# cmusphinx/pocketsphinx

Hardware: NVIDIA H100
Metric: frames/sec senone-eval+Viterbi (higher is better)
Workload: dtype f32->i16/i32

## Files before the change

### include/psb200.h

```cpp
#ifndef PSB200_H
#define PSB200_H

#include <stddef.h>
#include <stdint.h>

#ifdef __cplusplus
extern "C" {
#endif

#define PSB_ABI_VERSION 2

typedef enum psb_status_e {
    PSB_OK = 0,
    PSB_ERR_ARG = -1,
    PSB_ERR_CUDA = -2,
    PSB_ERR_NOMEM = -3,
    PSB_ERR_STATE = -4
} psb_status_t;

enum { PSB_KIND_PTM = 0, PSB_KIND_SEMI = 1, PSB_KIND_MS = 2 };

#define PSB_MAX_FEAT 8
#define PSB_MAX_TOPN 8
#define PSB_HMM_MAX_NSTATE 5
// ... 6 lines not shown
typedef struct psb_model_desc_s {
    int32_t kind, n_sen, n_mgau, n_feat, n_density, topn;
    int32_t featlen[PSB_MAX_FEAT];
    int32_t ds_ratio;
    int32_t aw;
    int32_t logadd_ms_size, logadd_ms_zero;
    int32_t on_device;
    const float *mean, *var, *det;
    const uint8_t *mixw, *mixw_cb;
    const int32_t *sen2cb;
    const uint8_t *logadd8;
    const uint32_t *logadd_ms;
    const uint8_t *topn_beam;
    int32_t fixed_point;
} psb_model_desc_t;

typedef struct psb_model_s psb_model_t;

int psb_model_create(const psb_model_desc_t *desc, int device, psb_model_t **out);
void psb_model_free(psb_model_t *m);
int psb_model_update_gaussians(psb_model_t *m, const float *mean, const float *var, const float *det);
int psb_model_n_sen(const psb_model_t *m);
int psb_model_device(const psb_model_t *m);

typedef struct psb_scorer_s psb_scorer_t;

int psb_scorer_create(psb_model_t *m, int32_t n_hist, psb_scorer_t **out);
void psb_scorer_free(psb_scorer_t *s);
int psb_scorer_reset(psb_scorer_t *s);
int psb_scorer_set_frame_idx(psb_scorer_t *s, int32_t frame_idx);
int32_t psb_scorer_get_frame_idx(const psb_scorer_t *s);
int psb_scorer_frame_eval(psb_scorer_t *s, int16_t *senscr, const uint8_t *senone_active,
                          int32_t n_senone_active, const float *const *feat, int32_t frame,
                          int32_t compallsen);

typedef struct psb_batch_s psb_batch_t;

int psb_batch_create(psb_model_t *m, int32_t max_utts, int64_t max_frames, psb_batch_t **out);
void psb_batch_free(psb_batch_t *b);
int psb_batch_score_host(psb_batch_t *b, const float *feats, const int32_t *utt_off,
                         int32_t n_utt, int16_t *senscr);
int psb_batch_score_device(psb_batch_t *b, const float *d_feats, const int32_t *utt_off,
                           int32_t n_utt, int16_t *d_senscr);
int psb_batch_sync(psb_batch_t *b);
int16_t *psb_batch_senscr_device(psb_batch_t *b);
int psb_batch_last_kernel_ms(psb_batch_t *b, float *out3);
int psb_batch_event_record(psb_batch_t *b, int slot);
int psb_batch_event_elapsed_ms(psb_batch_t *b, float *ms);
int psb_batch_tc_check(psb_batch_t *b, float *ratio, int32_t *max_candidates, int64_t *stats4);
#define PSB_TC_N_COUNTERS 15
int psb_batch_tc_counters(psb_batch_t *b, int64_t *out, int32_t n);
#define PSB_MS_PLAN_N 14
int psb_batch_ms_plan(psb_batch_t *b, int64_t total_frames, int64_t *out, int32_t n);
#define PSB_TM_PLAN_N 5
int psb_batch_tm_plan(psb_batch_t *b, int64_t total_frames, int64_t *out, int32_t n);
int psb_batch_get_topn(psb_batch_t *b, int32_t *rec, int64_t n_frames);

typedef struct psb_hmm_s {
    void *ctx;
    int32_t score[PSB_HMM_MAX_NSTATE];
    int32_t history[PSB_HMM_MAX_NSTATE];
    int32_t out_score;
    int32_t out_history;
    uint16_t ssid;
    uint16_t senid[PSB_HMM_MAX_NSTATE];
    int32_t bestscore;
    int16_t tmatid;
    int32_t frame;
    uint8_t mpx;
    uint8_t n_emit_state;
} psb_hmm_t;

typedef struct psb_hmmctx_s psb_hmmctx_t;

int psb_hmmctx_create(int32_t n_emit_state, const uint8_t *tp, int32_t n_tmat,
                      const uint16_t *sseq, int32_t n_sseq, int32_t n_sen, int device,
                      psb_hmmctx_t **out);
void psb_hmmctx_free(psb_hmmctx_t *c);

int psb_hmm_vit_eval_batch(psb_hmmctx_t *c, psb_hmm_t *hmms, int32_t n, const int16_t *senscr,
                           int32_t *best);
int psb_hmm_vit_eval_ptrs(psb_hmmctx_t *c, psb_hmm_t *const *hmms, int32_t n,
                          const int16_t *senscr, int32_t *best);

typedef struct psb_hmmset_s psb_hmmset_t;
int psb_hmmset_create(psb_hmmctx_t *c, int64_t n_max, int32_t n_seg_max, psb_hmmset_t **out);
void psb_hmmset_free(psb_hmmset_t *s);
int psb_hmmset_upload(psb_hmmset_t *s, const psb_hmm_t *hmms, int64_t n, const int64_t *seg_off,
                      int32_t n_seg);
int psb_hmmset_download(psb_hmmset_t *s, psb_hmm_t *hmms);
int psb_hmmset_eval_frames_device(psb_hmmset_t *s, const int16_t *d_senscr, const int64_t *d_row0,
                                  const int32_t *d_n_rows, int32_t n_frames, int32_t *d_best,
                                  float *ms);
int psb_hmmset_sweep_device(psb_hmmset_t *s, const int16_t *d_senscr, int64_t rows_total,
                            const int64_t *d_row0, const int32_t *d_n_rows, int32_t n_frames,
                            int32_t *d_best, float *ms);
int psb_hmmset_sweep_beam_device(psb_hmmset_t *s, const int16_t *d_senscr, int64_t rows_total,
                                 const int64_t *d_row0, const int32_t *d_n_rows, int32_t n_frames,
                                 int32_t frame0, int32_t beam, int32_t maxhmmpf, int32_t *d_best,
                                 int32_t *d_n_active, float *ms);
int psb_hmmset_use_batch_stream(psb_hmmset_t *s, psb_batch_t *b);
int psb_hmmset_snapshot(psb_hmmset_t *s);
int psb_hmmset_restore(psb_hmmset_t *s);
int psb_hmmset_eval_host(psb_hmmset_t *s, const int16_t *senscr, int32_t *best);

typedef struct psb_phoneloop_s psb_phoneloop_t;

// ... 256 lines not shown
```

### pocketsphinx_b200/api.py

```python
import ctypes as C

import numpy as np

from . import _lib
from ._lib import ModelDesc, PsbError, check, lib
from .model import PackedModel

KIND_ID = {"ptm": 0, "s2_semi": 1, "ms": 2}

HMM_DTYPE = np.dtype({
    "names": ["ctx", "score", "history", "out_score", "out_history", "ssid", "senid",
              "bestscore", "tmatid", "frame", "mpx", "n_emit_state"],
    "formats": ["<u8", ("<i4", 5), ("<i4", 5), "<i4", "<i4", "<u2", ("<u2", 5),
                "<i4", "<i2", "<i4", "u1", "u1"],
    "offsets": [0, 8, 28, 48, 52, 56, 58, 68, 72, 76, 80, 81],
    "itemsize": 88,
})


def _p(a):
    if a is None:
        return None
    if hasattr(a, "data_ptr"):
        return a.data_ptr()
# ... 131 lines not shown

    def set_pipeline(self, n):
        check(lib().psb_batch_set_pipeline(self.h, int(n)), "psb_batch_set_pipeline")

    def event_record(self, slot):
        check(lib().psb_batch_event_record(self.h, slot), "psb_batch_event_record")

    def event_elapsed_ms(self):
        ms = C.c_float()
        check(lib().psb_batch_event_elapsed_ms(self.h, C.byref(ms)), "psb_batch_event_elapsed_ms")
        return ms.value

    def run_phoneloop_device(self, phoneloop, utt_off, d_best_ptr=None, d_pen_ptr=None):
        utt_off = np.ascontiguousarray(utt_off, np.int32)
        check(lib().psb_phoneloop_run_device(phoneloop.h, self.senscr_device_ptr(), _p(utt_off), len(utt_off) - 1,
                                             d_best_ptr, d_pen_ptr, None, self.h), "psb_phoneloop_run_device")

    def decode_device(self, phoneloop, d_feats_ptr, utt_off):
        utt_off = np.ascontiguousarray(utt_off, np.int32)
        pb, pp = C.c_void_p(), C.c_void_p()
        check(lib().psb_decode_batch_device(self.h, phoneloop.h, d_feats_ptr, _p(utt_off), len(utt_off) - 1,
                                            C.byref(pb), C.byref(pp)), "psb_decode_batch_device")
        return pb.value, pp.value

    def get_topn(self, n_frames):
        rec = np.zeros((n_frames, self.model.pm.n_mgau * self.model.pm.n_feat, 4), np.int32)
        check(lib().psb_batch_get_topn(self.h, _p(rec), n_frames), "psb_batch_get_topn")
        return rec

    TC_COUNTERS = ("rows", "from_filter_alone", "exact_distances", "tie_fixups", "over_cap", "lane_over",
                   "fallback_listed", "fallback_all", "split_lists", "fail_gap", "fail_straddle", "fail_sign",
                   "fail_saturation", "tiles_per_cta", "ctas_per_pair")

    def tc_check(self):
        r, n = C.c_float(), C.c_int32()
        check(lib().psb_batch_tc_check(self.h, C.byref(r), C.byref(n), None), "psb_batch_tc_check")
        st = np.zeros(len(self.TC_COUNTERS), np.int64)
        check(lib().psb_batch_tc_counters(self.h, _p(st), len(st)), "psb_batch_tc_counters")
        self.tc_stats = {k: int(v) for k, v in zip(self.TC_COUNTERS, st)}
        return r.value, n.value

    MS_PLAN = ("tile", "fuse", "prefetch", "nt", "n_used", "all", "frames_per_cta", "tiles_x", "chunk", "n_chunks",
               "dist_bytes", "n_sm", "transposed", "tile_smem")

    def ms_plan(self, total_frames):
        v = np.zeros(len(self.MS_PLAN), np.int64)
        check(lib().psb_batch_ms_plan(self.h, int(total_frames), _p(v), len(v)), "psb_batch_ms_plan")
        return {k: int(x) for k, x in zip(self.MS_PLAN, v)}

    TM_TOPN = ("tc_filter", "ptm_scan", "ptm_scalar", "semi_split", "fixed")
    TM_SENONE = ("ptm_senone4", "ptm_senone_8b", "ptm_senone_4b", "semi_senone4", "semi_senone_8b", "semi_senone_4b")

    def tm_plan(self, total_frames):
        v = np.zeros(5, np.int64)
        check(lib().psb_batch_tm_plan(self.h, int(total_frames), _p(v), len(v)), "psb_batch_tm_plan")
        return dict(topn="+".join(n for i, n in enumerate(self.TM_TOPN) if int(v[0]) >> i & 1),
                    senone=self.TM_SENONE[int(v[1])], threads=int(v[2]), n_bsen=int(v[3]), smem=int(v[4]))

    def decode_host(self, phoneloop, feats, utt_off, want_senscr=False, best=None, pen=None, senscr=None):
        pm = self.model.pm
        utt_off = np.ascontiguousarray(utt_off, np.int32)
        total = int(utt_off[-1])
        if best is None:
            best = np.zeros(total, np.int32)
        if pen is None:
            pen = np.zeros((total, phoneloop.n_phones), np.int32)
        if want_senscr and senscr is None:
            senscr = np.zeros((total, pm.n_sen), np.int16)
        check(lib().psb_decode_batch_host(self.h, phoneloop.h, _p(feats), _p(utt_off), len(utt_off) - 1,
                                          _p(best), _p(pen), _p(senscr) if want_senscr else None),
              "psb_decode_batch_host")
        return (best, pen, senscr) if want_senscr else (best, pen)

    def decode_pcm_host(self, fe, phoneloop, pcm, samp_off, want_senscr=False):
        pm = self.model.pm
        pcm = np.ascontiguousarray(pcm, np.int16)
        samp_off = np.ascontiguousarray(samp_off, np.int64)
        n_utt = len(samp_off) - 1
        total = sum(fe.n_frames(int(samp_off[u + 1] - samp_off[u])) for u in range(n_utt))
        frame_off = np.zeros(n_utt + 1, np.int32)
        best = np.zeros(total, np.int32)
        pen = np.zeros((total, phoneloop.n_phones), np.int32)
        senscr = np.zeros((total, pm.n_sen), np.int16) if want_senscr else None
        check(lib().psb_decode_batch_pcm_host(self.h, fe.h, phoneloop.h, _p(pcm) if pcm.size else None, _p(samp_off), n_utt,
                                              _p(frame_off), _p(best), _p(pen), _p(senscr) if want_senscr else None),
              "psb_decode_batch_pcm_host")
        return (frame_off, best, pen, senscr) if want_senscr else (frame_off, best, pen)

    def score_pcm(self, fe, pcm, samp_off):
        pcm = np.ascontiguousarray(pcm, np.int16)
        samp_off = np.ascontiguousarray(samp_off, np.int64)
        n_utt = len(samp_off) - 1
        frame_off = np.zeros(n_utt + 1, np.int32)
        check(lib().psb_fe_process_host(fe.h, _p(pcm) if pcm.size else None, _p(samp_off), n_utt, None, None,
                                        _p(frame_off)), "psb_fe_process_host")
        if frame_off[-1]:
            self.score_device(lib().psb_fe_device_feats(fe.h), frame_off)
            self.sync()
        return frame_off

    def close(self):
        if self.h:
            lib().psb_batch_free(self.h)
            self.h = None


class HmmContext:

    def __init__(self, tp, sseq, n_sen, device=0):
        self.tp = np.ascontiguousarray(tp, np.uint8)
# ... 761 lines not shown
```

### pocketsphinx_b200/csrc/psb_ptm.cu

```cuda
#include "psb_gau.cuh"
#include "psb_internal.cuh"
#include "psb_tm.cuh"

#include <string.h>

#include <algorithm>
#include <numeric>

namespace {

constexpr int TOPN_WARPS = 4;
constexpr int MAX_NDW = 8;

template <int FL, bool SEMI>
__device__ __forceinline__ int gau_dist_fx(const float4 *__restrict__ r, const float (&x)[FL], int *dmin)
{
    constexpr int RECF = (1 + 2 * FL + 3) / 4 * 4;
    int rr[RECF];
#pragma unroll
    for (int q = 0; q < RECF / 4; ++q) {
        float4 v = r[q];
        rr[4 * q + 0] = __float_as_int(v.x); rr[4 * q + 1] = __float_as_int(v.y);
        rr[4 * q + 2] = __float_as_int(v.z); rr[4 * q + 3] = __float_as_int(v.w);
    }
// ... 544 lines not shown
    uint8_t *cb16 = tab + PSB_LOGADD8_N;
    int16_t *asc = reinterpret_cast<int16_t *>(cb16 + 16);
    const long long frame = blockIdx.x;
    const int tid = threadIdx.x;

    for (int i = tid; i < PSB_LOGADD8_N; i += blockDim.x) tab[i] = logadd_tab[i];
    if (FOURBIT && tid < 16) cb16[tid] = mixw_cb[tid];
    if (tid < n_feat) norm[tid] = PSB_WORST_SCORE;
    __syncthreads();
    ptm_norm_rows<false>(topn, frame, K, n_feat, nd, mixw_stride, norm, rowoff, nsc, nullptr);
    __syncthreads();

    int best = 0x7fffffff;
    for (int s = tid; s < n_sen; s += blockDim.x) {
        const int i0 = (int)sen2cb[s] * n_feat;
        const uint8_t *__restrict__ mw = mixw + (FOURBIT ? (s >> 1) : s);
        int ascore = 0;
        for (int f = 0; f < n_feat; ++f)
            ascore += ptm_mix<FOURBIT>(mw, rowoff[i0 + f], nsc[i0 + f], tab, cb16);
        best = min(best, ascore);
        asc[s] = (int16_t)ascore;
    }
    store_relative_to_best(best, red, asc, senscr + frame * n_sen, n_sen);
}

template <bool FOURBIT>
__global__ void __launch_bounds__(256)
semi_senone_kernel(const int4 *__restrict__ topn, const uint8_t *__restrict__ mixw,
                   const uint8_t *__restrict__ mixw_cb, const uint8_t *__restrict__ logadd_tab,
                   int16_t *__restrict__ senscr, int n_sen, int n_feat, int nd, int mixw_stride)
{
    extern __shared__ int smem_i[];
    uint4 *rowoff = reinterpret_cast<uint4 *>(smem_i);
    uint4 *nsc = rowoff + n_feat;
    uint8_t *tab = reinterpret_cast<uint8_t *>(nsc + n_feat);
    uint8_t *cb16 = tab + PSB_LOGADD8_N;
    __shared__ int cnt[PSB_MAX_FEAT];
    const long long frame = blockIdx.x;
    const int tid = threadIdx.x;
    for (int i = tid; i < PSB_LOGADD8_N; i += blockDim.x) tab[i] = logadd_tab[i];
    if (FOURBIT && tid < 16) cb16[tid] = mixw_cb[tid];
    semi_rows<false>(topn, frame, n_feat, nd, mixw_stride, rowoff, nsc, nullptr, cnt);
    __syncthreads();
    const int s = blockIdx.y * blockDim.x + tid;
    if (s >= n_sen) return;
    int16_t acc = 0;
    if (!FOURBIT || s < (n_sen & ~1)) {
        for (int f = 0; f < n_feat; ++f)
            acc = (int16_t)(acc + semi_mix<FOURBIT>(mixw, s, rowoff[f], nsc[f], cnt[f], tab, cb16));
    }
    senscr[frame * n_sen + s] = acc;
}

__global__ void __launch_bounds__(512)
ptm_senone4_kernel(const int4 *__restrict__ topn, const uint8_t *__restrict__ mixw,
                   const uint16_t *__restrict__ sen2cb, const int16_t *__restrict__ quadcb,
                   const int32_t *__restrict__ bsen, int n_bsen, const uint8_t *__restrict__ logadd_tab,
                   int16_t *__restrict__ senscr, int n_sen, int n_feat, int nd, int K, int mixw_stride)
{
    extern __shared__ int smem_i[];
    uint4 *rowoff = reinterpret_cast<uint4 *>(smem_i);
    uint4 *nsc = rowoff + K;
    uint4 *nvp = nsc + K;
    int *norm = reinterpret_cast<int *>(nvp + K);
    int *red = norm + 8;
    uint8_t *tab = reinterpret_cast<uint8_t *>(red + 32);
    int16_t *asc = reinterpret_cast<int16_t *>(tab + PSB_LOGADD8_N + 16);
    const long long frame = blockIdx.x;
    const int tid = threadIdx.x;

    for (int i = tid; i < PSB_LOGADD8_N; i += blockDim.x) tab[i] = logadd_tab[i];
    if (tid < n_feat) norm[tid] = PSB_WORST_SCORE;
    __syncthreads();
    ptm_norm_rows<true>(topn, frame, K, n_feat, nd, mixw_stride, norm, rowoff, nsc, nvp);
    __syncthreads();

    int best = 0x7fffffff;
    const int n_quads = (n_sen + 3) >> 2;
    for (int q = tid; q < n_quads; q += blockDim.x) {
        const int c = quadcb[q];
        if (c < 0) continue;
        const int s0 = q << 2, i0 = c * n_feat;
        const uint8_t *mw = mixw + s0;
        unsigned acc01 = 0u, acc23 = 0u;
        for (int f = 0; f < n_feat; ++f) {
            const uint4 ro = rowoff[i0 + f], nv = nvp[i0 + f];
            const unsigned w0 = *reinterpret_cast<const unsigned *>(mw + ro.x);
            const unsigned w1 = *reinterpret_cast<const unsigned *>(mw + ro.y);
            const unsigned w2 = *reinterpret_cast<const unsigned *>(mw + ro.z);
            const unsigned w3 = *reinterpret_cast<const unsigned *>(mw + ro.w);
            unsigned x01 = __byte_perm(w0, 0u, 0x4140) + nv.x;
            unsigned x23 = __byte_perm(w0, 0u, 0x4342) + nv.x;
            x01 = logadd8_16x2(tab, x01, w1, 0x4140, nv.y); x23 = logadd8_16x2(tab, x23, w1, 0x4342, nv.y);
            x01 = logadd8_16x2(tab, x01, w2, 0x4140, nv.z); x23 = logadd8_16x2(tab, x23, w2, 0x4342, nv.z);
            x01 = logadd8_16x2(tab, x01, w3, 0x4140, nv.w); x23 = logadd8_16x2(tab, x23, w3, 0x4342, nv.w);
            acc01 += x01;
            acc23 += x23;
        }
        const int unbias = n_feat * SEN_BIAS;
        const int a0 = (int)(acc01 & 0xffffu) - unbias, a1 = (int)(acc01 >> 16) - unbias;
        const int a2 = (int)(acc23 & 0xffffu) - unbias, a3 = (int)(acc23 >> 16) - unbias;
        best = min(min(best, a0), min(min(a1, a2), a3));
        *reinterpret_cast<short4 *>(asc + s0) = make_short4((short)a0, (short)a1, (short)a2, (short)a3);
    }
    for (int i = tid; i < n_bsen; i += blockDim.x) {
        const int s = bsen[i];
        const int i0 = (int)sen2cb[s] * n_feat;
        int ascore = 0;
        for (int f = 0; f < n_feat; ++f)
            ascore += ptm_mix<false>(mixw + s, rowoff[i0 + f], nsc[i0 + f], tab, nullptr);
        best = min(best, ascore);
        asc[s] = (int16_t)ascore;
    }
    store_relative_to_best(best, red, asc, senscr + frame * n_sen, n_sen);
}

template <int FL>
int launch_topnq(psb_batch_t *b, const int32_t *d_klist, int n_k, const GroupTabs &tabs, int n_groups,
                 const int32_t *d_featoff)
{
    psb_model_t *m = b->m;
    constexpr int RECF2 = (2 + 4 * FL + 3) / 4 * 4;
    const size_t smem = (size_t)(m->n_density / 2) * RECF2 * sizeof(float) + (size_t)QCAP * TOPN_WARPS * 32 * sizeof(float);
    auto kern = ptm_topnq_kernel<FL>;
    PSB_CUDA(cudaFuncSetAttribute(kern, cudaFuncAttributeMaxDynamicSharedMemorySize, (int)smem));
    dim3 grid(n_k, (n_groups + TOPN_WARPS - 1) / TOPN_WARPS);
    kern<<<grid, TOPN_WARPS * 32, smem, b->stream>>>(m->d_rec2, m->d_rec2_off, d_klist, b->d_featT, tabs, b->d_topn, n_groups,
                                                    m->n_density, m->n_feat, m->sumlen, d_featoff, m->K, m->ds_ratio);
    PSB_LAUNCH_CHECK();
    return PSB_OK;
}

template <int FL, bool SEMI>
int launch_topn(psb_batch_t *b, const int32_t *d_klist, int n_k, const GroupTabs &tabs, int n_groups,
                const int32_t *d_featoff)
{
    psb_model_t *m = b->m;
    if constexpr (!SEMI && FL <= 16) {
        if (!m->fixed_point) return launch_topnq<FL>(b, d_klist, n_k, tabs, n_groups, d_featoff);
    }
    auto kern = ptm_topn_kernel<FL, SEMI, true>;
    if constexpr (!SEMI && FL > 16) {
        if (!m->fixed_point) kern = ptm_topn_kernel<FL, false, false>;
    }
    size_t smem = (size_t)m->n_density * rec_floats(FL) * sizeof(float);
    PSB_CUDA(cudaFuncSetAttribute(kern, cudaFuncAttributeMaxDynamicSharedMemorySize, (int)smem));
    const int warps = (long long)n_k * ((n_groups + TOPN_WARPS - 1) / TOPN_WARPS) >= 4 * psb_sm_count(m->device) ? TOPN_WARPS : 1;
    dim3 grid(n_k, (n_groups + warps - 1) / warps);
    kern<<<grid, warps * 32, smem, b->stream>>>(m->d_rec, m->d_rec_off, d_klist, b->d_featT, tabs, b->d_topn, n_groups,
                                               m->n_density, m->n_feat, m->sumlen, d_featoff, m->K, m->ds_ratio,
                                               m->d_topn_beam);
    PSB_LAUNCH_CHECK();
    return PSB_OK;
}

__global__ void __launch_bounds__(512)
semi_senone4_kernel(const int4 *__restrict__ topn, const uint8_t *__restrict__ mixw,
                    const uint8_t *__restrict__ logadd_tab, int16_t *__restrict__ senscr, int n_sen, int n_feat, int nd,
                    int mixw_stride)
{
    __shared__ uint4 rowoff[PSB_MAX_FEAT], nvp[PSB_MAX_FEAT], nsc[PSB_MAX_FEAT];
    __shared__ int cnt[PSB_MAX_FEAT];
    __shared__ uint8_t tab[PSB_LOGADD8_N];
    const long long frame = blockIdx.x;
    const int tid = threadIdx.x;
    for (int i = tid; i < PSB_LOGADD8_N; i += blockDim.x) tab[i] = logadd_tab[i];
    semi_rows<true>(topn, frame, n_feat, nd, mixw_stride, rowoff, nsc, nvp, cnt);
    __syncthreads();
    int16_t *dst = senscr + frame * n_sen;
    const int n_quads = n_sen >> 2;
    for (int q = tid; q < n_quads; q += blockDim.x) {
        const int s0 = q << 2;
        const uint8_t *mw = mixw + s0;
        short a0 = 0, a1 = 0, a2 = 0, a3 = 0;
        for (int f = 0; f < n_feat; ++f) {
            const uint4 ro = rowoff[f], nv = nvp[f];
            const int n = cnt[f];
            const unsigned w0 = *reinterpret_cast<const unsigned *>(mw + ro.x);
            unsigned x01 = __byte_perm(w0, 0u, 0x4140) + nv.x, x23 = __byte_perm(w0, 0u, 0x4342) + nv.x;
            if (n > 1) {
                const unsigned w1 = *reinterpret_cast<const unsigned *>(mw + ro.y);
                x01 = logadd8_16x2(tab, x01, w1, 0x4140, nv.y); x23 = logadd8_16x2(tab, x23, w1, 0x4342, nv.y);
            }
            if (n > 2) {
                const unsigned w2 = *reinterpret_cast<const unsigned *>(mw + ro.z);
                x01 = logadd8_16x2(tab, x01, w2, 0x4140, nv.z); x23 = logadd8_16x2(tab, x23, w2, 0x4342, nv.z);
            }
            if (n > 3) {
                const unsigned w3 = *reinterpret_cast<const unsigned *>(mw + ro.w);
                x01 = logadd8_16x2(tab, x01, w3, 0x4140, nv.w); x23 = logadd8_16x2(tab, x23, w3, 0x4342, nv.w);
            }
            a0 = (short)(a0 + (int)(x01 & 0xffffu) - SEN_BIAS);
            a1 = (short)(a1 + (int)(x01 >> 16) - SEN_BIAS);
            a2 = (short)(a2 + (int)(x23 & 0xffffu) - SEN_BIAS);
            a3 = (short)(a3 + (int)(x23 >> 16) - SEN_BIAS);
        }
        if ((((uintptr_t)(dst + s0)) & 7) == 0)
            *reinterpret_cast<short4 *>(dst + s0) = make_short4(a0, a1, a2, a3);
        else { dst[s0] = a0; dst[s0 + 1] = a1; dst[s0 + 2] = a2; dst[s0 + 3] = a3; }
    }
    for (int s = (n_quads << 2) + tid; s < n_sen; s += blockDim.x) {
        int16_t acc = 0;
        for (int f = 0; f < n_feat; ++f)
            acc = (int16_t)(acc + semi_mix<false>(mixw, s, rowoff[f], nsc[f], cnt[f], tab, nullptr));
        dst[s] = acc;
    }
}

enum TmTopn { TOPN_TC_FILTER, TOPN_PTM_SCAN, TOPN_PTM_SCALAR, TOPN_SEMI_SPLIT, TOPN_FIXED };
enum TmSenone { SEN_PTM4, SEN_PTM_8B, SEN_PTM_4B, SEN_SEMI4, SEN_SEMI_8B, SEN_SEMI_4B };

bool topn_fl_instantiated(int fl)
{
    for (int v : {13, 12, 24, 3, 39, 1, 2, 4, 8, 16, 26, 32})
        if (fl == v) return true;
    return false;
}

constexpr size_t TM_SMEM_MAX = 227 * 1024;

struct TmPlan {
    unsigned topn_paths;
    bool semi_split;
    int senone;
    int threads;
    size_t smem;
};

int tm_plan(const psb_model_t *m, TmPlan *p)
{
    PSB_REQUIRE(m->kind == PSB_KIND_PTM || m->kind == PSB_KIND_SEMI, "psb_launch_ptm_batch: model is neither PTM nor semi-continuous");
    const bool semi = m->kind == PSB_KIND_SEMI;
    PSB_REQUIRE(m->topn == TOPN, "tied-mixture batch kernels are built for -topn 4 (got %d)", m->topn);
    PSB_REQUIRE(m->n_density % 32 == 0 && m->n_density <= 32 * MAX_NDW,
                "PTM batch kernels need n_density in {32..256, multiple of 32} (got %d)", m->n_density);
    const int K = m->K;
    const bool use_tc = !semi && psb_tc_usable(m);
    p->semi_split = semi && !m->fixed_point;
    p->topn_paths = 0;
    for (int f = 0; f < m->n_feat; ++f) {
        const int fl = m->featlen[f];
        if (use_tc) { p->topn_paths |= 1u << TOPN_TC_FILTER; continue; }
        if (!topn_fl_instantiated(fl)) {
            psb_set_error("no %s instantiation for stream length %d", p->semi_split ? "semi_dist_kernel" : "ptm_topn_kernel", fl);
            return PSB_ERR_ARG;
        }
        int path;
        if (p->semi_split) path = TOPN_SEMI_SPLIT;
        else if (m->fixed_point) path = TOPN_FIXED;
        else path = fl <= 16 ? TOPN_PTM_SCAN : TOPN_PTM_SCALAR;
        p->topn_paths |= 1u << path;
    }
    const bool bias_ok = (TOPN - 1) * m->logadd8_max < SEN_BIAS;
    if (semi) {
        PSB_REQUIRE(K <= 512, "semi_senone_kernel handles at most 512 streams (got %d)", K);
        if (!m->mixw_4bit && bias_ok) {
            p->senone = SEN_SEMI4; p->threads = 512; p->smem = 0;
        }
        else {
            p->senone = m->mixw_4bit ? SEN_SEMI_4B : SEN_SEMI_8B;
            p->threads = 256;
            p->smem = (size_t)K * 32 + PSB_LOGADD8_N + 16;
        }
        return PSB_OK;
    }
    PSB_REQUIRE(K <= 512, "ptm_senone_kernel handles at most 512 (codebook, stream) pairs (got %d)", K);
    PSB_REQUIRE((size_t)m->n_feat * m->n_density * m->mixw_stride < (1ull << 32), "mixture-weight table too large for 32-bit offsets");
    const size_t smem = (size_t)K * 32 + 8 * 4 + 32 * 4 + PSB_LOGADD8_N + 16 + (size_t)m->n_sen * 2;
    if (m->mixw_4bit || !bias_ok) {
        p->senone = m->mixw_4bit ? SEN_PTM_4B : SEN_PTM_8B;
        p->threads = 512;
        p->smem = smem;
    }
    else {
        const int n_quads = (m->n_sen + 3) / 4;
        const int iters = (n_quads + 511) / 512;
        p->senone = SEN_PTM4;
        p->threads = std::min(512, std::max(std::max(256, roundup(K, 32)), roundup((n_quads + iters - 1) / iters, 32)));
        p->smem = smem + 8 + (size_t)K * 16;
    }
    PSB_REQUIRE(p->smem <= TM_SMEM_MAX, "%d senones do not fit the PTM senone kernel's shared memory (%zu bytes, at most %zu)",
                m->n_sen, p->smem, TM_SMEM_MAX);
    return PSB_OK;
}

}

extern "C" int psb_batch_tm_plan(psb_batch_t *b, int64_t total_frames, int64_t *out, int32_t n)
{
    PSB_REQUIRE(b && (out || n == 0) && n >= 0 && total_frames >= 0, "psb_batch_tm_plan: bad argument");
    TmPlan p;
    const int rc = tm_plan(b->m, &p);
    if (rc) return rc;
    const int64_t v[PSB_TM_PLAN_N] = {p.topn_paths, p.senone, p.threads, b->m->n_bsen, (int64_t)p.smem};
    memcpy(out, v, sizeof(int64_t) * (size_t)std::min<int32_t>(n, PSB_TM_PLAN_N));
    return PSB_OK;
}

int psb_launch_ptm_batch(psb_batch_t *b, const float *d_feats, const int32_t *utt_off, int32_t n_utt,
                         int16_t *d_senscr)
{
    psb_model_t *m = b->m;
    TmPlan plan;
    int rc = tm_plan(m, &plan);
    if (rc) return rc;
    const bool semi = m->kind == PSB_KIND_SEMI;
    const long long total = utt_off[n_utt];
    PSB_REQUIRE(n_utt <= b->max_utts && total <= b->max_frames, "batch too large for this psb_batch_t");
    b->last_frames = total;
    if (total == 0 || n_utt == 0) return PSB_OK;
    const int D = m->sumlen, K = m->K;

    std::vector<int> perm(n_utt);
    std::iota(perm.begin(), perm.end(), 0);
    std::stable_sort(perm.begin(), perm.end(), [&](int a, int c) {
        return utt_off[a + 1] - utt_off[a] > utt_off[c + 1] - utt_off[c];
    });
    const int n_groups = (n_utt + 31) / 32;
    size_t n32 = (size_t)n_groups * 64 + n_groups + K + PSB_MAX_FEAT;
    n32 = (n32 + 1) & ~(size_t)1;
    size_t need = n32 + 2 * (size_t)(2 * n_groups + 1);
    rc = b->d_tab.reserve(need, need);
    if (!rc) rc = b->h_tab.reserve(need, need);
    if (rc) return rc;
    int32_t *lane_len = b->h_tab, *lane_off = lane_len + n_groups * 32, *grp_maxT = lane_off + n_groups * 32;
    int32_t *klist = grp_maxT + n_groups, *featoff = klist + K;
    long long *grp_base = reinterpret_cast<long long *>(b->h_tab + n32), *warp_base = grp_base + n_groups;
    long long featT_floats = 0, items = 0;
    for (int g = 0; g < n_groups; ++g) {
        int mx = 0;
        for (int l = 0; l < 32; ++l) {
            int idx = g * 32 + l;
            if (idx < n_utt) {
                int u = perm[idx];
                lane_len[idx] = utt_off[u + 1] - utt_off[u];
                lane_off[idx] = utt_off[u];
                mx = std::max(mx, lane_len[idx]);
            }
            else { lane_len[idx] = 0; lane_off[idx] = 0; }
        }
        grp_maxT[g] = mx;
        grp_base[g] = featT_floats;
        warp_base[g] = items;
        featT_floats += (long long)mx * D * 32;
        items += mx;
    }
    warp_base[n_groups] = items;
    for (int f = 0; f < PSB_MAX_FEAT; ++f) featoff[f] = f < m->n_feat ? m->featoff[f] : 0;
    const bool use_tc = plan.topn_paths == 1u << TOPN_TC_FILTER, semi_split = plan.semi_split;
    const bool scan = !use_tc && !semi_split;
    if (scan && (rc = b->d_featT.reserve((size_t)featT_floats, (size_t)featT_floats >> 3))) return rc;
    std::vector<std::vector<int>> byfl;
    std::vector<int> fls;
    for (int f = 0; f < m->n_feat; ++f) {
        size_t i = std::find(fls.begin(), fls.end(), m->featlen[f]) - fls.begin();
        if (i == fls.size()) { fls.push_back(m->featlen[f]); byfl.emplace_back(); }
        for (int cb = 0; cb < m->n_mgau; ++cb) byfl[i].push_back(cb * m->n_feat + f);
    }
    {
        int pos = 0;
        for (auto &v : byfl) for (int k : v) klist[pos++] = k;
    }
    PSB_CUDA(cudaMemcpyAsync(b->d_tab, b->h_tab, need * sizeof(int32_t), cudaMemcpyHostToDevice, b->stream));
    GroupTabs tabs;
    tabs.lane_len = b->d_tab;
    tabs.lane_off = b->d_tab + n_groups * 32;
    tabs.grp_maxT = b->d_tab + n_groups * 64;
    const int32_t *d_klist = b->d_tab + n_groups * 64 + n_groups, *d_featoff = d_klist + K;
    tabs.grp_base = reinterpret_cast<const long long *>(b->d_tab + n32);
    const long long *d_warp_base = tabs.grp_base + n_groups;

    PSB_CUDA(cudaEventRecord(b->ev[0], b->stream));
    if (scan) {
        int warps = 8;
        while (warps > 1 && (size_t)warps * 32 * (D + 1) * sizeof(float) > 48 * 1024) warps >>= 1;
        size_t smem = (size_t)warps * 32 * (D + 1) * sizeof(float);
        PSB_REQUIRE(smem <= 48 * 1024, "feature vectors of %d floats are too long for transpose_feats_kernel", D);
        long long blocks = (items + warps - 1) / warps;
        transpose_feats_kernel<<<(unsigned)blocks, warps * 32, smem, b->stream>>>(
            d_feats, b->d_featT, tabs, d_warp_base, n_groups, D);
        PSB_LAUNCH_CHECK();
    }
    PSB_CUDA(cudaEventRecord(b->ev[1], b->stream));
    if (use_tc) {
        rc = psb_launch_ptm_tc(b, d_feats, utt_off, n_utt, d_klist, d_featoff);
        if (rc) return rc;
    }
    else if (semi_split) {
        const size_t need_d = (size_t)K * total * m->n_density;
        if ((rc = b->d_semi_dist.reserve(need_d, need_d / 8)) || (rc = b->d_uttoff.reserve((size_t)n_utt + 1, 64))) return rc;
        PSB_CUDA(cudaMemcpyAsync(b->d_uttoff, utt_off, ((size_t)n_utt + 1) * sizeof(int32_t), cudaMemcpyHostToDevice, b->stream));
        PSB_REQUIRE(total <= 0x7fffffffLL, "too many frames for one launch");
        int pos = 0;
        for (size_t i = 0; i < fls.size(); ++i) {
            const int n_k = (int)byfl[i].size();
            const dim3 grid((unsigned)total, (unsigned)n_k);
            switch (fls[i]) {
#define CASE(FL) case FL: semi_dist_kernel<FL><<<grid, roundup(m->n_density, 32), 0, b->stream>>>(                     \
                    m->d_rec, m->d_rec_off, d_klist + pos, d_feats, b->d_semi_dist, total, m->n_density, m->n_feat, D, d_featoff); break;
                CASE(13) CASE(12) CASE(24) CASE(3) CASE(39) CASE(1) CASE(2) CASE(4) CASE(8) CASE(16) CASE(26) CASE(32)
#undef CASE
// ... 5 lines not shown
            pos += n_k;
        }
        const int warps = 4;
        const unsigned blocks = (unsigned)(((long long)n_utt * K + warps - 1) / warps);
        switch (m->n_density / 32) {
#define CASE(NDW) case NDW: semi_scan_kernel<NDW><<<blocks, warps * 32, 0, b->stream>>>(                              \
                    b->d_semi_dist, b->d_uttoff, n_utt, K, total, m->n_density, m->ds_ratio, m->d_topn_beam, b->d_topn); break;
            CASE(1) CASE(2) CASE(3) CASE(4) CASE(5) CASE(6) CASE(7) CASE(8)
#undef CASE
        }
        PSB_LAUNCH_CHECK();
    }
    else {
        int pos = 0;
        for (size_t i = 0; i < fls.size(); ++i) {
            int n_k = (int)byfl[i].size(), rc;
            switch (fls[i]) {
#define CASE(FL) case FL: rc = semi ? launch_topn<FL, true>(b, d_klist + pos, n_k, tabs, n_groups, d_featoff) \
                                   : launch_topn<FL, false>(b, d_klist + pos, n_k, tabs, n_groups, d_featoff); break;
                CASE(13) CASE(12) CASE(24) CASE(3) CASE(39) CASE(1) CASE(2) CASE(4) CASE(8) CASE(16) CASE(26) CASE(32)
#undef CASE
            default:
                psb_set_error("no ptm_topn_kernel instantiation for stream length %d", fls[i]);
                return PSB_ERR_ARG;
            }
            if (rc) return rc;
            pos += n_k;
        }
    }
    PSB_CUDA(cudaEventRecord(b->ev[2], b->stream));
    if (semi) {
        PSB_REQUIRE(total <= 65535LL * 32768, "too many frames for one launch");
        const dim3 grid((unsigned)total, (m->n_sen + plan.threads - 1) / plan.threads);
        if (plan.senone == SEN_SEMI4)
            semi_senone4_kernel<<<(unsigned)total, plan.threads, 0, b->stream>>>(b->d_topn, m->d_mixw, m->d_logadd8, d_senscr,
                                                                               m->n_sen, m->n_feat, m->n_density, m->mixw_stride);
        else if (plan.senone == SEN_SEMI_4B)
            semi_senone_kernel<true><<<grid, plan.threads, plan.smem, b->stream>>>(
                b->d_topn, m->d_mixw, m->d_mixw_cb, m->d_logadd8, d_senscr, m->n_sen, m->n_feat, m->n_density, m->mixw_stride);
        else
            semi_senone_kernel<false><<<grid, plan.threads, plan.smem, b->stream>>>(
                b->d_topn, m->d_mixw, m->d_mixw_cb, m->d_logadd8, d_senscr, m->n_sen, m->n_feat, m->n_density, m->mixw_stride);
        PSB_LAUNCH_CHECK();
    }
    else {
        if (plan.senone == SEN_PTM_4B || plan.senone == SEN_PTM_8B) {
            auto kern = plan.senone == SEN_PTM_4B ? ptm_senone_kernel<true> : ptm_senone_kernel<false>;
            PSB_CUDA(cudaFuncSetAttribute(kern, cudaFuncAttributeMaxDynamicSharedMemorySize, (int)plan.smem));
            kern<<<(unsigned)total, plan.threads, plan.smem, b->stream>>>(
                b->d_topn, m->d_mixw, m->d_mixw_cb, m->d_sen2cb, m->d_logadd8, d_senscr, m->n_sen, m->n_feat,
                m->n_density, K, m->mixw_stride);
        }
        else {
            PSB_CUDA(cudaFuncSetAttribute(ptm_senone4_kernel, cudaFuncAttributeMaxDynamicSharedMemorySize, (int)plan.smem));
            ptm_senone4_kernel<<<(unsigned)total, plan.threads, plan.smem, b->stream>>>(
                b->d_topn, m->d_mixw, m->d_sen2cb, m->d_quadcb, m->d_bsen, m->n_bsen, m->d_logadd8, d_senscr, m->n_sen,
                m->n_feat, m->n_density, K, m->mixw_stride);
        }
        PSB_LAUNCH_CHECK();
    }
    PSB_CUDA(cudaEventRecord(b->ev[3], b->stream));
    return PSB_OK;
}
```

### pocketsphinx_b200/csrc/psb_tm.cuh

```cuda
#pragma once
#include "psb_internal.cuh"

namespace {

constexpr int TOPN = 4;
constexpr int SEN_BIAS = 64;

__device__ __forceinline__ int logadd8(const uint8_t *tab, int x, int y)
{
    return min(x, y) - tab[abs(x - y)];
}

__device__ __forceinline__ unsigned logadd8_16x2(const uint8_t *tab, unsigned x, unsigned w, unsigned sel, unsigned nvj)
{
    const unsigned y = __byte_perm(w, 0u, sel);
    const unsigned mn = __viaddmin_u16x2(y, nvj, x);
    const unsigned mx = __viaddmax_u16x2(y, nvj, x);
    const unsigned d = mx - mn;
    const unsigned t = (unsigned)tab[d & 0xffffu] | ((unsigned)tab[d >> 16] << 16);
    return mn - t;
}

__device__ __forceinline__ int ptm_weight4(const uint8_t *cb16, int b)
{
    return cb16[(b & 1) ? b >> 4 : b & 0x0f];
}
__device__ __forceinline__ int semi_weight4(const uint8_t *cb16, int b, int s)
{
    return cb16[(s & 1) ? b >> 4 : b & 0x0f];
}

__device__ __forceinline__ unsigned tm_row(unsigned cwb, int j, int f, int nd, int mixw_stride)
{
    return ((unsigned)f * nd + ((cwb >> (8 * j)) & 0xff)) * (unsigned)mixw_stride;
}

__device__ __forceinline__ uint4 sen_bias16x2(const unsigned (&nv)[TOPN])
{
    return make_uint4((nv[0] + SEN_BIAS) * 0x10001u, (nv[1] + SEN_BIAS) * 0x10001u,
                      (nv[2] + SEN_BIAS) * 0x10001u, (nv[3] + SEN_BIAS) * 0x10001u);
}

template <bool X2>
__device__ __forceinline__ void ptm_norm_rows(const int4 *__restrict__ topn, long long frame, int K, int n_feat, int nd,
                                              int mixw_stride, int *norm, uint4 *rowoff, uint4 *nsc, uint4 *nvp)
{
    const int tid = threadIdx.x;
    int4 r = make_int4(0, 0, 0, 0);
    if (tid < K) {
        r = topn[frame * K + tid];
        atomicMax(&norm[tid % n_feat], r.x);
    }
    __syncthreads();
    if (tid < K) {
        const int f = tid % n_feat;
        const int base = norm[f] - r.x;
        const unsigned eb = (unsigned)r.z, cwb = (unsigned)r.y;
        unsigned ro[TOPN], nv[TOPN];
#pragma unroll
        for (int j = 0; j < TOPN; ++j) {
            int v = base + (int)((eb >> (8 * j)) & 0xff);
            nv[j] = (unsigned)(v > PSB_MAX_NEG_ASCR ? PSB_MAX_NEG_ASCR : v);
            ro[j] = tm_row(cwb, j, f, nd, mixw_stride);
        }
        rowoff[tid] = make_uint4(ro[0], ro[1], ro[2], ro[3]);
        nsc[tid] = make_uint4(nv[0], nv[1], nv[2], nv[3]);
        if (X2) nvp[tid] = sen_bias16x2(nv);
    }
}

template <bool X2>
__device__ __forceinline__ void semi_rows(const int4 *__restrict__ topn, long long frame, int n_feat, int nd,
                                          int mixw_stride, uint4 *rowoff, uint4 *nsc, uint4 *nvp, int *cnt)
{
    const int tid = threadIdx.x;
    if (tid < n_feat) {
        const int4 r = topn[frame * n_feat + tid];
        const unsigned cwb = (unsigned)r.y, eb = (unsigned)r.z;
        unsigned ro[TOPN], nv[TOPN];
#pragma unroll
        for (int j = 0; j < TOPN; ++j) {
            ro[j] = tm_row(cwb, j, tid, nd, mixw_stride);
            nv[j] = (eb >> (8 * j)) & 0xff;
        }
        rowoff[tid] = make_uint4(ro[0], ro[1], ro[2], ro[3]);
        nsc[tid] = make_uint4(nv[0], nv[1], nv[2], nv[3]);
        if (X2) nvp[tid] = sen_bias16x2(nv);
        cnt[tid] = r.x;
    }
}

template <bool FOURBIT>
__device__ __forceinline__ int ptm_mix(const uint8_t *__restrict__ mw, uint4 ro, uint4 nv, const uint8_t *tab,
                                       const uint8_t *cb16)
{
    int w0 = mw[ro.x], w1 = mw[ro.y], w2 = mw[ro.z], w3 = mw[ro.w];
    if (FOURBIT) {
        w0 = ptm_weight4(cb16, w0); w1 = ptm_weight4(cb16, w1);
        w2 = ptm_weight4(cb16, w2); w3 = ptm_weight4(cb16, w3);
    }
    int fden = w0 + (int)nv.x;
    fden = logadd8(tab, fden, w1 + (int)nv.y);
    fden = logadd8(tab, fden, w2 + (int)nv.z);
    fden = logadd8(tab, fden, w3 + (int)nv.w);
    return fden;
}

template <bool FOURBIT>
__device__ __forceinline__ int semi_mix(const uint8_t *__restrict__ mixw, int s, uint4 ro, uint4 nv, int n,
                                        const uint8_t *tab, const uint8_t *cb16)
{
    const unsigned rr[TOPN] = {ro.x, ro.y, ro.z, ro.w}, vv[TOPN] = {nv.x, nv.y, nv.z, nv.w};
    int tmp = 0;
#pragma unroll
    for (int k = 0; k < TOPN; ++k) {
        if (k == 0 || k < n) {
            const int w = FOURBIT ? semi_weight4(cb16, mixw[rr[k] + (unsigned)(s >> 1)], s) : mixw[rr[k] + (unsigned)s];
            const int v = w + (int)vv[k];
            tmp = k == 0 ? v : logadd8(tab, tmp, v);
        }
    }
// ... 22 lines not shown
```

Before: 12.74 million.

## Process runs of consecutive frames per CTA and reuse mixture-weight loads across frames

```diff
diff --git a/include/psb200.h b/include/psb200.h
--- a/include/psb200.h
+++ b/include/psb200.h
@@ -82,7 +82,7 @@
 int psb_batch_tc_counters(psb_batch_t *b, int64_t *out, int32_t n);
 #define PSB_MS_PLAN_N 14
 int psb_batch_ms_plan(psb_batch_t *b, int64_t total_frames, int64_t *out, int32_t n);
-#define PSB_TM_PLAN_N 5
+#define PSB_TM_PLAN_N 7
 int psb_batch_tm_plan(psb_batch_t *b, int64_t total_frames, int64_t *out, int32_t n);
 int psb_batch_get_topn(psb_batch_t *b, int32_t *rec, int64_t n_frames);
 
diff --git a/pocketsphinx_b200/api.py b/pocketsphinx_b200/api.py
--- a/pocketsphinx_b200/api.py
+++ b/pocketsphinx_b200/api.py
@@ -207,10 +207,11 @@
     TM_SENONE = ("ptm_senone4", "ptm_senone_8b", "ptm_senone_4b", "semi_senone4", "semi_senone_8b", "semi_senone_4b")
 
     def tm_plan(self, total_frames):
-        v = np.zeros(5, np.int64)
+        v = np.zeros(7, np.int64)
         check(lib().psb_batch_tm_plan(self.h, int(total_frames), _p(v), len(v)), "psb_batch_tm_plan")
         return dict(topn="+".join(n for i, n in enumerate(self.TM_TOPN) if int(v[0]) >> i & 1),
-                    senone=self.TM_SENONE[int(v[1])], threads=int(v[2]), n_bsen=int(v[3]), smem=int(v[4]))
+                    senone=self.TM_SENONE[int(v[1])], threads=int(v[2]), n_bsen=int(v[3]), smem=int(v[4]),
+                    run=int(v[5]), quads=int(v[6]))
 
     def decode_host(self, phoneloop, feats, utt_off, want_senscr=False, best=None, pen=None, senscr=None):
         pm = self.model.pm
diff --git a/pocketsphinx_b200/csrc/psb_ptm.cu b/pocketsphinx_b200/csrc/psb_ptm.cu
--- a/pocketsphinx_b200/csrc/psb_ptm.cu
+++ b/pocketsphinx_b200/csrc/psb_ptm.cu
@@ -620,11 +620,58 @@
     senscr[frame * n_sen + s] = acc;
 }
 
-__global__ void __launch_bounds__(512)
-ptm_senone4_kernel(const int4 *__restrict__ topn, const uint8_t *__restrict__ mixw,
-                   const uint16_t *__restrict__ sen2cb, const int16_t *__restrict__ quadcb,
-                   const int32_t *__restrict__ bsen, int n_bsen, const uint8_t *__restrict__ logadd_tab,
-                   int16_t *__restrict__ senscr, int n_sen, int n_feat, int nd, int K, int mixw_stride)
+__device__ __forceinline__ unsigned carry_map(unsigned prev, unsigned cur)
+{
+    unsigned m = 0;
+#pragma unroll
+    for (int j = 0; j < TOPN; ++j) {
+        const unsigned eq = __vcmpeq4(prev, ((cur >> (8 * j)) & 0xffu) * 0x01010101u);
+        m |= (eq ? (unsigned)(__ffs(eq) - 1) >> 3 : 0xffu) << (8 * j);
+    }
+    return m;
+}
+
+__device__ __forceinline__ void quad_chain(const uint8_t *tab, const unsigned (&w)[TOPN], uint4 nv, unsigned &acc01,
+                                           unsigned &acc23)
+{
+    unsigned x01 = __byte_perm(w[0], 0u, 0x4140) + nv.x;
+    unsigned x23 = __byte_perm(w[0], 0u, 0x4342) + nv.x;
+    x01 = logadd8_16x2(tab, x01, w[1], 0x4140, nv.y); x23 = logadd8_16x2(tab, x23, w[1], 0x4342, nv.y);
+    x01 = logadd8_16x2(tab, x01, w[2], 0x4140, nv.z); x23 = logadd8_16x2(tab, x23, w[2], 0x4342, nv.z);
+    x01 = logadd8_16x2(tab, x01, w[3], 0x4140, nv.w); x23 = logadd8_16x2(tab, x23, w[3], 0x4342, nv.w);
+    acc01 += x01;
+    acc23 += x23;
+}
+
+__device__ __forceinline__ void quad_store(unsigned acc01, unsigned acc23, int n_feat, int s0, int16_t *asc, int &best)
+{
+    const int unbias = n_feat * SEN_BIAS;
+    const int a0 = (int)(acc01 & 0xffffu) - unbias, a1 = (int)(acc01 >> 16) - unbias;
+    const int a2 = (int)(acc23 & 0xffffu) - unbias, a3 = (int)(acc23 >> 16) - unbias;
+    best = min(best, min(min(a0, a1), min(a2, a3)));
+    *reinterpret_cast<short4 *>(asc + s0) = make_short4((short)a0, (short)a1, (short)a2, (short)a3);
+}
+
+__device__ __forceinline__ unsigned load_word(const uint8_t *__restrict__ mw, unsigned off)
+{
+    return *reinterpret_cast<const unsigned *>(mw + off);
+}
+
+__device__ __forceinline__ void quad_chain_loaded(const uint8_t *__restrict__ mixw, const uint8_t *tab, const uint4 *rowoff,
+                                                  const uint4 *nvp, int p, int s0, unsigned &acc01, unsigned &acc23)
+{
+    const uint4 ro = rowoff[p];
+    const unsigned w[TOPN] = {load_word(mixw + s0, ro.x), load_word(mixw + s0, ro.y), load_word(mixw + s0, ro.z),
+                              load_word(mixw + s0, ro.w)};
+    quad_chain(tab, w, nvp[p], acc01, acc23);
+}
+
+template <int Q, int NF, int MINB, bool DIAG>
+__global__ void __launch_bounds__(512, MINB)
+ptm_senone_run_kernel(const int4 *__restrict__ topn, const int2 *__restrict__ runs, const uint8_t *__restrict__ mixw,
+                      const uint16_t *__restrict__ sen2cb, const int16_t *__restrict__ quadcb,
+                      const int32_t *__restrict__ bsen, int n_bsen, const uint8_t *__restrict__ logadd_tab,
+                      int16_t *__restrict__ senscr, int n_sen, int n_feat, int nd, int K, int mixw_stride)
 {
     extern __shared__ int smem_i[];
     uint4 *rowoff = reinterpret_cast<uint4 *>(smem_i);
@@ -632,55 +679,86 @@
     uint4 *nvp = nsc + K;
     int *norm = reinterpret_cast<int *>(nvp + K);
     int *red = norm + 8;
-    uint8_t *tab = reinterpret_cast<uint8_t *>(red + 32);
+    unsigned *cmap = reinterpret_cast<unsigned *>(red + 32);
+    uint8_t *tab = reinterpret_cast<uint8_t *>(cmap + ((K + 1) & ~1));
     int16_t *asc = reinterpret_cast<int16_t *>(tab + PSB_LOGADD8_N + 16);
-    const long long frame = blockIdx.x;
     const int tid = threadIdx.x;
+    const int2 run = runs[blockIdx.x];
+    const int n_quads = (n_sen + 3) >> 2;
 
     for (int i = tid; i < PSB_LOGADD8_N; i += blockDim.x) tab[i] = logadd_tab[i];
-    if (tid < n_feat) norm[tid] = PSB_WORST_SCORE;
-    __syncthreads();
-    ptm_norm_rows<true>(topn, frame, K, n_feat, nd, mixw_stride, norm, rowoff, nsc, nvp);
-    __syncthreads();
-
-    int best = 0x7fffffff;
-    const int n_quads = (n_sen + 3) >> 2;
-    for (int q = tid; q < n_quads; q += blockDim.x) {
-        const int c = quadcb[q];
-        if (c < 0) continue;
-        const int s0 = q << 2, i0 = c * n_feat;
-        const uint8_t *mw = mixw + s0;
-        unsigned acc01 = 0u, acc23 = 0u;
-        for (int f = 0; f < n_feat; ++f) {
-            const uint4 ro = rowoff[i0 + f], nv = nvp[i0 + f];
-            const unsigned w0 = *reinterpret_cast<const unsigned *>(mw + ro.x);
-            const unsigned w1 = *reinterpret_cast<const unsigned *>(mw + ro.y);
-            const unsigned w2 = *reinterpret_cast<const unsigned *>(mw + ro.z);
-            const unsigned w3 = *reinterpret_cast<const unsigned *>(mw + ro.w);
-            unsigned x01 = __byte_perm(w0, 0u, 0x4140) + nv.x;
-            unsigned x23 = __byte_perm(w0, 0u, 0x4342) + nv.x;
-            x01 = logadd8_16x2(tab, x01, w1, 0x4140, nv.y); x23 = logadd8_16x2(tab, x23, w1, 0x4342, nv.y);
-            x01 = logadd8_16x2(tab, x01, w2, 0x4140, nv.z); x23 = logadd8_16x2(tab, x23, w2, 0x4342, nv.z);
-            x01 = logadd8_16x2(tab, x01, w3, 0x4140, nv.w); x23 = logadd8_16x2(tab, x23, w3, 0x4342, nv.w);
-            acc01 += x01;
-            acc23 += x23;
-        }
-        const int unbias = n_feat * SEN_BIAS;
-        const int a0 = (int)(acc01 & 0xffffu) - unbias, a1 = (int)(acc01 >> 16) - unbias;
-        const int a2 = (int)(acc23 & 0xffffu) - unbias, a3 = (int)(acc23 >> 16) - unbias;
-        best = min(min(best, a0), min(min(a1, a2), a3));
-        *reinterpret_cast<short4 *>(asc + s0) = make_short4((short)a0, (short)a1, (short)a2, (short)a3);
-    }
-    for (int i = tid; i < n_bsen; i += blockDim.x) {
-        const int s = bsen[i];
-        const int i0 = (int)sen2cb[s] * n_feat;
-        int ascore = 0;
-        for (int f = 0; f < n_feat; ++f)
-            ascore += ptm_mix<false>(mixw + s, rowoff[i0 + f], nsc[i0 + f], tab, nullptr);
-        best = min(best, ascore);
-        asc[s] = (int16_t)ascore;
-    }
-    store_relative_to_best(best, red, asc, senscr + frame * n_sen, n_sen);
+    int cb[Q];
+    unsigned w[Q][NF][TOPN];
+#pragma unroll
+    for (int i = 0; i < Q; ++i) {
+        const int q = tid + i * (int)blockDim.x;
+        cb[i] = q < n_quads ? quadcb[q] : -1;
+    }
+    unsigned prev_cw = 0u;
+
+    for (int t = 0; t < run.y; ++t) {
+        const long long frame = (long long)run.x + t;
+        if (tid < n_feat) norm[tid] = PSB_WORST_SCORE;
+        __syncthreads();
+        const unsigned cw = ptm_norm_rows<true>(topn, frame, K, n_feat, nd, mixw_stride, norm, rowoff, nsc, nvp);
+        if (tid < K) {
+            cmap[tid] = t == 0 ? 0xffffffffu : carry_map(prev_cw, cw);
+            prev_cw = cw;
+        }
+        __syncthreads();
+
+        int best = 0x7fffffff;
+#pragma unroll
+        for (int i = 0; i < Q; ++i) {
+            if (cb[i] < 0) continue;
+            const int s0 = (tid + i * (int)blockDim.x) << 2;
+            unsigned acc01 = 0u, acc23 = 0u;
+#pragma unroll
+            for (int f = 0; f < NF; ++f) {
+                if (f >= n_feat) break;
+                const int p = cb[i] * n_feat + f;
+                unsigned (&ww)[TOPN] = w[i][f];
+                if (!DIAG || t == 0) {
+                    const unsigned m = cmap[p];
+                    uint4 ro = make_uint4(0, 0, 0, 0);
+                    if (m & 0x80808080u) ro = rowoff[p];
+                    const unsigned rr[TOPN] = {ro.x, ro.y, ro.z, ro.w};
+                    unsigned nw[TOPN];
+#pragma unroll
+                    for (int j = 0; j < TOPN; ++j) {
+                        const unsigned sel = (m >> (8 * j)) & 0xffu;
+                        if (sel & 0x80u) nw[j] = load_word(mixw + s0, rr[j]);
+                        else {
+                            const unsigned a = (sel & 1u) ? ww[1] : ww[0], b = (sel & 1u) ? ww[3] : ww[2];
+                            nw[j] = (sel & 2u) ? b : a;
+                        }
+                    }
+#pragma unroll
+                    for (int j = 0; j < TOPN; ++j) ww[j] = nw[j];
+                }
+                quad_chain(tab, ww, nvp[p], acc01, acc23);
+            }
+            for (int f = NF; f < n_feat; ++f) quad_chain_loaded(mixw, tab, rowoff, nvp, cb[i] * n_feat + f, s0, acc01, acc23);
+            quad_store(acc01, acc23, n_feat, s0, asc, best);
+        }
+        for (int q = tid + Q * (int)blockDim.x; q < n_quads; q += blockDim.x) {
+            const int c = quadcb[q];
+            if (c < 0) continue;
+            unsigned acc01 = 0u, acc23 = 0u;
+            for (int f = 0; f < n_feat; ++f) quad_chain_loaded(mixw, tab, rowoff, nvp, c * n_feat + f, q << 2, acc01, acc23);
+            quad_store(acc01, acc23, n_feat, q << 2, asc, best);
+        }
+        for (int i = tid; i < n_bsen; i += blockDim.x) {
+            const int s = bsen[i];
+            const int i0 = (int)sen2cb[s] * n_feat;
+            int ascore = 0;
+            for (int f = 0; f < n_feat; ++f)
+                ascore += ptm_mix<false>(mixw + s, rowoff[i0 + f], nsc[i0 + f], tab, nullptr);
+            best = min(best, ascore);
+            asc[s] = (int16_t)ascore;
+        }
+        store_relative_to_best(best, red, asc, senscr + frame * n_sen, n_sen);
+    }
 }
 
 template <int FL>
@@ -787,12 +865,17 @@
 
 constexpr size_t TM_SMEM_MAX = 227 * 1024;
 
+constexpr int PTM_RUN_FRAMES = 16;
+constexpr int PTM_RUN_QUADS = 3, PTM_RUN_STREAMS = 3, PTM_RUN_MINB = 1;
+
 struct TmPlan {
     unsigned topn_paths;
     bool semi_split;
     int senone;
     int threads;
     size_t smem;
+    int run;
+    int quads;
 };
 
 int tm_plan(const psb_model_t *m, TmPlan *p)
@@ -806,6 +889,8 @@
     const bool use_tc = !semi && psb_tc_usable(m);
     p->semi_split = semi && !m->fixed_point;
     p->topn_paths = 0;
+    p->run = 1;
+    p->quads = 0;
     for (int f = 0; f < m->n_feat; ++f) {
         const int fl = m->featlen[f];
         if (use_tc) { p->topn_paths |= 1u << TOPN_TC_FILTER; continue; }
@@ -845,10 +930,39 @@
         const int iters = (n_quads + 511) / 512;
         p->senone = SEN_PTM4;
         p->threads = std::min(512, std::max(std::max(256, roundup(K, 32)), roundup((n_quads + iters - 1) / iters, 32)));
-        p->smem = smem + 8 + (size_t)K * 16;
+        p->smem = smem + 8 + (size_t)K * 16 + (size_t)((K + 1) & ~1) * 4;
+        p->run = PTM_RUN_FRAMES;
+        p->quads = (n_quads + p->threads - 1) / p->threads;
     }
     PSB_REQUIRE(p->smem <= TM_SMEM_MAX, "%d senones do not fit the PTM senone kernel's shared memory (%zu bytes, at most %zu)",
                 m->n_sen, p->smem, TM_SMEM_MAX);
+    return PSB_OK;
+}
+
+int count_runs(const int32_t *utt_off, int n_utt, int R)
+{
+    long long n = 0;
+    for (int u = 0; u < n_utt; ++u) n += (utt_off[u + 1] - utt_off[u] + R - 1) / R;
+    return (int)n;
+}
+
+void build_runs(const int32_t *utt_off, int n_utt, int R, int2 *runs, int n_runs)
+{
+    int r = 0;
+    for (int u = 0; u < n_utt && r < n_runs; ++u)
+        for (int f = utt_off[u]; f < utt_off[u + 1]; f += R) runs[r++] = make_int2(f, std::min(R, utt_off[u + 1] - f));
+}
+
+template <int Q, int NF, int MINB, bool DIAG>
+int launch_senone_runs(psb_batch_t *b, const int2 *d_runs, int n_runs, int threads, size_t smem, int16_t *d_senscr)
+{
+    psb_model_t *m = b->m;
+    auto kern = ptm_senone_run_kernel<Q, NF, MINB, DIAG>;
+    PSB_CUDA(cudaFuncSetAttribute(kern, cudaFuncAttributeMaxDynamicSharedMemorySize, (int)smem));
+    kern<<<(unsigned)n_runs, threads, smem, b->stream>>>(b->d_topn, d_runs, m->d_mixw, m->d_sen2cb, m->d_quadcb, m->d_bsen,
+                                                        m->n_bsen, m->d_logadd8, d_senscr, m->n_sen, m->n_feat,
+                                                        m->n_density, m->K, m->mixw_stride);
+    PSB_LAUNCH_CHECK();
     return PSB_OK;
 }
 
@@ -860,10 +974,44 @@
     TmPlan p;
     const int rc = tm_plan(b->m, &p);
     if (rc) return rc;
-    const int64_t v[PSB_TM_PLAN_N] = {p.topn_paths, p.senone, p.threads, b->m->n_bsen, (int64_t)p.smem};
+    const int64_t v[PSB_TM_PLAN_N] = {p.topn_paths, p.senone, p.threads, b->m->n_bsen, (int64_t)p.smem, p.run, p.quads};
     memcpy(out, v, sizeof(int64_t) * (size_t)std::min<int32_t>(n, PSB_TM_PLAN_N));
     return PSB_OK;
 }
+
+#ifdef PSB_SENONE_CANDIDATES
+extern "C" int psb_ptm_senone_candidate(psb_batch_t *b, const int32_t *utt_off, int32_t n_utt, int32_t quads, int32_t minb, int32_t diag,
+                                        int32_t run, int32_t max_threads, int16_t *d_out, float *ms)
+{
+    psb_model_t *m = b->m;
+    TmPlan plan;
+    int rc = tm_plan(m, &plan);
+    if (rc) return rc;
+    PSB_REQUIRE(plan.senone == SEN_PTM4 && run >= 1 && max_threads >= 256 && max_threads <= 512 && d_out && ms,
+                "psb_ptm_senone_candidate: bad argument");
+    const int n_quads = (m->n_sen + 3) / 4, iters = (n_quads + max_threads - 1) / max_threads;
+    const int threads = std::min(max_threads, std::max(std::max(256, roundup(m->K, 32)), roundup((n_quads + iters - 1) / iters, 32)));
+    const int n_runs = count_runs(utt_off, n_utt, run);
+    std::vector<int2> h_runs(n_runs);
+    build_runs(utt_off, n_utt, run, h_runs.data(), n_runs);
+    DevBuf<int2> d_runs;
+    PSB_CUDA(cudaSetDevice(m->device));
+    if ((rc = d_runs.reserve((size_t)n_runs))) return rc;
+    PSB_CUDA(cudaMemcpy(d_runs, h_runs.data(), sizeof(int2) * (size_t)n_runs, cudaMemcpyHostToDevice));
+    PSB_CUDA(cudaEventRecord(b->ev[2], b->stream));
+    if (diag) rc = launch_senone_runs<PTM_RUN_QUADS, PTM_RUN_STREAMS, PTM_RUN_MINB, true>(b, d_runs, n_runs, threads, plan.smem, d_out);
+    else if (quads == 0) rc = launch_senone_runs<PTM_RUN_QUADS, PTM_RUN_STREAMS, PTM_RUN_MINB, false>(b, d_runs, n_runs, threads, plan.smem, d_out);
+    else if (quads == 3 && minb == 2) rc = launch_senone_runs<3, 3, 2, false>(b, d_runs, n_runs, threads, plan.smem, d_out);
+    else if (quads == 2 && minb == 2) rc = launch_senone_runs<2, 3, 2, false>(b, d_runs, n_runs, threads, plan.smem, d_out);
+    else if (quads == 2 && minb == 1) rc = launch_senone_runs<2, 3, 1, false>(b, d_runs, n_runs, threads, plan.smem, d_out);
+    else if (quads == 4 && minb == 1) rc = launch_senone_runs<4, 3, 1, false>(b, d_runs, n_runs, threads, plan.smem, d_out);
+    else rc = PSB_ERR_ARG;
+    PSB_CUDA(cudaEventRecord(b->ev[3], b->stream));
+    PSB_CUDA(cudaEventSynchronize(b->ev[3]));
+    PSB_CUDA(cudaEventElapsedTime(ms, b->ev[2], b->ev[3]));
+    return rc;
+}
+#endif
 
 int psb_launch_ptm_batch(psb_batch_t *b, const float *d_feats, const int32_t *utt_off, int32_t n_utt,
                          int16_t *d_senscr)
@@ -888,6 +1036,9 @@
     size_t n32 = (size_t)n_groups * 64 + n_groups + K + PSB_MAX_FEAT;
     n32 = (n32 + 1) & ~(size_t)1;
     size_t need = n32 + 2 * (size_t)(2 * n_groups + 1);
+    const size_t runs_at = need;
+    const int n_runs = plan.senone == SEN_PTM4 ? count_runs(utt_off, n_utt, plan.run) : 0;
+    need += 2 * (size_t)n_runs;
     rc = b->d_tab.reserve(need, need);
     if (!rc) rc = b->h_tab.reserve(need, need);
     if (rc) return rc;
@@ -915,6 +1066,7 @@
     }
     warp_base[n_groups] = items;
     for (int f = 0; f < PSB_MAX_FEAT; ++f) featoff[f] = f < m->n_feat ? m->featoff[f] : 0;
+    build_runs(utt_off, n_utt, plan.run, reinterpret_cast<int2 *>(b->h_tab + runs_at), n_runs);
     const bool use_tc = plan.topn_paths == 1u << TOPN_TC_FILTER, semi_split = plan.semi_split;
     const bool scan = !use_tc && !semi_split;
     if (scan && (rc = b->d_featT.reserve((size_t)featT_floats, (size_t)featT_floats >> 3))) return rc;
@@ -1026,10 +1178,9 @@
                 m->n_density, K, m->mixw_stride);
         }
         else {
-            PSB_CUDA(cudaFuncSetAttribute(ptm_senone4_kernel, cudaFuncAttributeMaxDynamicSharedMemorySize, (int)plan.smem));
-            ptm_senone4_kernel<<<(unsigned)total, plan.threads, plan.smem, b->stream>>>(
-                b->d_topn, m->d_mixw, m->d_sen2cb, m->d_quadcb, m->d_bsen, m->n_bsen, m->d_logadd8, d_senscr, m->n_sen,
-                m->n_feat, m->n_density, K, m->mixw_stride);
+            rc = launch_senone_runs<PTM_RUN_QUADS, PTM_RUN_STREAMS, PTM_RUN_MINB, false>(b, reinterpret_cast<const int2 *>(b->d_tab + runs_at), n_runs,
+                                                          plan.threads, plan.smem, d_senscr);
+            if (rc) return rc;
         }
         PSB_LAUNCH_CHECK();
     }
diff --git a/pocketsphinx_b200/csrc/psb_tm.cuh b/pocketsphinx_b200/csrc/psb_tm.cuh
--- a/pocketsphinx_b200/csrc/psb_tm.cuh
+++ b/pocketsphinx_b200/csrc/psb_tm.cuh
@@ -42,7 +42,7 @@
 }
 
 template <bool X2>
-__device__ __forceinline__ void ptm_norm_rows(const int4 *__restrict__ topn, long long frame, int K, int n_feat, int nd,
+__device__ __forceinline__ unsigned ptm_norm_rows(const int4 *__restrict__ topn, long long frame, int K, int n_feat, int nd,
                                               int mixw_stride, int *norm, uint4 *rowoff, uint4 *nsc, uint4 *nvp)
 {
     const int tid = threadIdx.x;
@@ -67,6 +67,7 @@
         nsc[tid] = make_uint4(nv[0], nv[1], nv[2], nv[3]);
         if (X2) nvp[tid] = sen_bias16x2(nv);
     }
+    return (unsigned)r.y;
 }
 
 template <bool X2>
```

New measurement: 9.791 million (median of 6 runs). 23.2% lower.
